# cshizhe/VLN-HAMT

Hardware: AMD Instinct MI355X
Metric: panorama-steps/sec, R2R proxy pretrain (36x768 views, 80-tok instr) (higher is better)
Workload: dtype bf16; 1 GPU; R2R 6-proxy-task pretrain step (fwd+bwd+clip+AdamW, dropout 0.1), fixed ViT features, R2R-canon model 174.8M params; per_gpu_batch=64, global_batch=64, txt_len=80, hist_len=5, views=36, task_mix=mlm:sap:sar:sprel:mrc:itm=5:1:1:1:2:2, parallelism=dp1, launch=hipGraph replay, dead_code_elimination=True

## Files before the change

### include/hamt.h

```cpp
#ifndef HAMT_H
#define HAMT_H

#include <stddef.h>
#include <stdint.h>

#ifdef __cplusplus
extern "C" {
#endif

#define HAMT_ABI_VERSION 2

typedef enum { HAMT_OK = 0, HAMT_ERR_ARG = -1, HAMT_ERR_UNSUPPORTED = -2, HAMT_ERR_LAUNCH = -3 } hamt_status;
typedef enum { HAMT_F32 = 0, HAMT_BF16 = 1,
               HAMT_U8G = 2,
               HAMT_F16 = 3 } hamt_dtype;
typedef enum { HAMT_PREC_BF16 = 0, HAMT_PREC_F32 = 1 } hamt_prec;

int hamt_version(void);
int hamt_last_error(char* buf, size_t n);
int hamt_last_kernel(char* buf, size_t n);
enum { HAMT_WS_GEMM_SPLITK = 0, HAMT_WS_COLSUM = 1, HAMT_WS_SUMSQ = 2, HAMT_WS_LN_BWD = 3, HAMT_WS_WGRAD_TABLE = 4, HAMT_WS_LNRED_TABLE = 5, HAMT_WS_VIS_EMBED_BWD = 6,
       HAMT_WS_EMBED_BWD = 7 ,
       HAMT_WS_OBJ_EMBED_BWD = 8, HAMT_WS_IMAGE_PREP = 9  };
size_t hamt_workspace_bytes(int op, const int* shape, int nshape);
// ... 196 lines not shown
  int layout;
  int ldy, dtype_y, Rpad;
} hamt_image_prep_desc;
int hamt_image_prep(const hamt_image_prep_desc* d, const hamt_image_view* views_host, const hamt_image_view* views_dev,
                    const uint8_t* src, const float* lut, void* y, void* ws, size_t ws_bytes, void* stream);
enum { HAMT_RESAMPLE_BICUBIC = 0 , HAMT_RESAMPLE_LANCZOS = 1  };
typedef struct {
  int n, H, W;
  int OH, OW;
  int x0, y0, w, h;
  int filter;
  int kx, ky;
} hamt_image_resample_desc;
int hamt_image_resample_taps(int in, int out, int filter, int first, int count, int32_t* xmin, int32_t* xcnt, int32_t* k, int ksize);
int hamt_image_resample(const hamt_image_resample_desc* d, const int32_t* xtab_host, const int32_t* ytab_host, const int32_t* xtab_dev,
                        const int32_t* ytab_dev, const uint8_t* src, uint8_t* dst, void* stream);
int hamt_add3(size_t n, const float* a, const float* b, const float* c, float* out, void* stream);
int hamt_dropout(size_t n, const float* x, float* y, float p, uint32_t call_id, const uint64_t* rng, void* stream);
int hamt_cast_f32_bf16(size_t n, const float* x, void* y, void* stream);
int hamt_unpack_padded(const void* src, const int32_t* prefix, int B, int maxlen, int row_bytes, int pad_byte, void* dst, void* stream);
int hamt_seq_masks(const int32_t* prefix, int add, int B, int maxlen, uint8_t* mask, int64_t* lens_out, void* stream);
int hamt_wire_pack_bf16(size_t n, const float* x, void* y, float scale, void* stream);
int hamt_wire_unpack_bf16(size_t n, const void* y, float* x, void* stream);
int hamt_fill_where_zero(size_t n, const int64_t* flag, float* x, float value, void* stream);
int hamt_extend_mask(size_t n, const void* mask_u8, float* out, void* stream);
int hamt_debug_fill_lds(uint32_t pattern, void* stream);
int hamt_debug_wgrad_timing(int on);
int hamt_debug_wgrad_times(float* us, int* tile_rows, double* flops, int cap);
int hamt_act_bwd(size_t n, const float* dy, const float* h, int mode, float* dx, void* stream);

int hamt_ce_fwd(int R, int C, const float* x, int ldx, const int64_t* label, float* loss, float* lse, void* stream);
int hamt_ce_bwd(int R, int C, const float* x, int ldx, const int64_t* label, const float* lse,
                const float* g, float* dx, int lddx, void* stream);
int hamt_mse_fwd(size_t n, const float* x, const float* t, float* loss, void* stream);
int hamt_mse_bwd(size_t n, const float* x, const float* t, const float* g, float* dx, void* stream);
int hamt_kl_fwd(int R, int C, const float* x, int ldx, const float* t, int ldt, float* loss, float* lse, void* stream);
int hamt_kl_bwd(int R, int C, const float* x, int ldx, const float* t, int ldt, const float* lse,
                const float* g, float* dx, int lddx, void* stream);
int hamt_eval_ce(int R, int C, const float* x, int ldx, const int64_t* label, float* ws, double* sums, int64_t* counts, void* stream);
int hamt_eval_kl(int R, int C, const float* x, int ldx, const float* t, int ldt, float* ws, double* sums, int64_t* counts,
                 void* stream);
int hamt_eval_mse_cols(int R, int C, const float* x, int ldx, const float* t, int ldt, double* sums, void* stream);
int hamt_a2c_fwd(int T, int B, const float* reward, const float* mask, const float* value, const float* logp, const float* ent,
                 const float* last_value, float gamma, float ent_w, float* ret, float* out, void* stream);
int hamt_a2c_bwd(int T, int B, const float* ret, const float* mask, const float* value, float ent_w, const float* g,
                 float* dlogp, float* dvalue, float* dent, void* stream);
#define HAMT_POLICY_TEACHER 0
#define HAMT_POLICY_ARGMAX 1
#define HAMT_POLICY_SAMPLE 2
int hamt_policy_step_fwd(int B, int V, int A, int mode, int64_t ignoreid, const float* logit, int ld_logit,
                         const int64_t* target, const uint8_t* bt_mask, const int32_t* cand_len, uint8_t* ended,
                         const float* ob_ang, const int64_t* forced_action, const float* uniform, const uint64_t* rng,
                         uint32_t call_id, float* ml, int64_t* action, float* logp, float* ent, float* mask,
                         int32_t* env_action, float* prev_angle, int32_t* hist_len, float* lse, void* stream);
int hamt_policy_step_bwd(int B, int V, int mode, int64_t ignoreid, const float* logit, int ld_logit, const int64_t* target,
                         const uint8_t* bt_mask, const int64_t* action, const float* lse, const float* g_ml,
                         const float* g_logp, const float* g_ent, int gs_ml, int gs_logp, int gs_ent, float* dlogit, int ld_dlogit,
                         void* stream);
#define HAMT_STOP_LOGIT_INDEX 0
#define HAMT_STOP_LOGIT_VALUE 1
int hamt_policy_ref_step_fwd(int B, int V, int O, int A, int mode, int stop_logit, int last_step, int64_t ignoreid,
                             const float* act_logit, int ld_act, const float* obj_logit, int ld_obj, const int32_t* obj_len,
                             const int32_t* cand_len, const int64_t* target, const int64_t* ref_target, const int32_t* obj_id,
                             const int32_t* goal_obj, const uint8_t* bt_mask, uint8_t* ended, const float* ob_ang,
                             const int64_t* forced_action, const float* uniform, const uint64_t* rng, uint32_t call_id,
                             float* ml, float* ref, int64_t* action, float* logp, float* ent, float* mask, int32_t* env_action,
// ... 90 lines not shown
```

### vln_hamt_amd/_lib.py

```python
from __future__ import annotations

import ctypes as C
import os

_HERE = os.path.dirname(os.path.abspath(__file__))
LIB_PATH = os.path.join(_HERE, "libhamt_hip.so")

HAMT_F32, HAMT_BF16, HAMT_U8G, HAMT_F16 = 0, 1, 2, 3
PREC_BF16, PREC_F32 = 0, 1
EPI_BIAS, EPI_GELU, EPI_RELU, EPI_ACCUM, EPI_MUL_DGELU, EPI_MUL_DRELU, EPI_SAVE_PRE = 1, 2, 4, 8, 16, 32, 64
EPI_GELU_GRAD, EPI_MUL_AUX, EPI_ADD_AUX, EPI_DROPOUT = 128, 256, 512, 1024
SUMSQ_SPARSE = 2
OPT_ADAMW, OPT_ADAM, OPT_RMSPROP, OPT_SGD = 0, 1, 2, 3

vp, i32, u32, f32, sz = C.c_void_p, C.c_int, C.c_uint32, C.c_float, C.c_size_t


class GemmDesc(C.Structure):
    _fields_ = [("M", i32), ("N", i32), ("K", i32), ("lda", i32), ("ldb", i32), ("ldc", i32), ("ldaux", i32),
                ("a_kmajor", i32), ("b_kmajor", i32), ("dtype_a", i32), ("dtype_b", i32), ("dtype_c", i32),
                ("dtype_aux", i32), ("prec", i32), ("epilogue", i32), ("alpha", f32), ("ka_rows", i32), ("kb_rows", i32),
                ("p_drop", f32), ("call_id", u32), ("rng", C.c_void_p)]


# ... 96 lines not shown
    "hamt_obj_embed_fwd": [C.POINTER(ObjEmbedDesc), C.POINTER(ObjEmbedParams)] + [vp] * 7,
    "hamt_obj_embed_bwd": [C.POINTER(ObjEmbedDesc), C.POINTER(ObjEmbedParams), C.POINTER(ObjEmbedGrads)] + [vp] * 10,
    "hamt_ln_fwd": [C.POINTER(LnDesc), vp, vp, vp, vp, vp, vp, vp, vp, vp, vp, vp],
    "hamt_ln_bwd": [C.POINTER(LnDesc), vp, vp, vp, vp, vp, vp, vp, vp, vp, vp, vp, vp, vp, vp],
    "hamt_ln_bwd_add": [C.POINTER(LnDesc), vp, vp, vp, vp, vp, vp, vp, vp, vp, vp, vp],
    "hamt_ln_bwd_reduce": [i32, i32, vp, vp, vp, vp, vp],
    "hamt_ln_bwd_reduce_grouped": [i32, vp, vp, sz, vp],
    "hamt_gather_rows": [i32, i32, vp, i32, vp, vp, i32, vp, i32, i32, vp],
    "hamt_scatter_add_rows": [i32, i32, vp, i32, i32, vp, vp, i32, vp],
    "hamt_scatter_add_rows_small": [i32, i32, vp, i32, i32, vp, i32, vp, vp, vp],
    "hamt_scatter_add_rows_ordered": [i32, i32, vp, i32, i32, vp, vp, i32, i32, vp, vp],
    "hamt_embed_sum_fwd": [i32, i32, i32, vp, vp, vp, vp, vp, vp],
    "hamt_embed_sum_bwd": [i32, i32, i32, i32, vp, vp, vp, vp, vp, vp, sz, vp],
    "hamt_mean_mid_fwd": [i32, i32, i32, vp, vp, vp],
    "hamt_mean_mid_bwd": [i32, i32, i32, vp, vp, vp],
    "hamt_mul_bcast_fwd": [i32, i32, i32, vp, vp, i32, vp, vp],
    "hamt_mul_bcast_bwd": [i32, i32, i32, vp, vp, i32, vp, vp, vp, vp],
    "hamt_sum_rows": [i32, i32, i32, vp, i32, vp, vp, vp],
    "hamt_patchify": [i32, i32, i32, i32, i32, vp, vp, i32, i32, i32, vp],
    "hamt_image_prep": [C.POINTER(ImagePrepDesc), vp, vp, vp, vp, vp, vp, sz, vp],
    "hamt_image_resample_taps": [i32, i32, i32, i32, i32, vp, vp, vp, i32],
    "hamt_image_resample": [C.POINTER(ImageResampleDesc), vp, vp, vp, vp, vp, vp, vp],
    "hamt_add3": [sz, vp, vp, vp, vp, vp],
    "hamt_dropout": [sz, vp, vp, f32, u32, vp, vp],
    "hamt_cast_f32_bf16": [sz, vp, vp, vp],
    "hamt_unpack_padded": [vp, vp, i32, i32, i32, i32, vp, vp],
    "hamt_seq_masks": [vp, i32, i32, i32, vp, vp, vp],
    "hamt_wire_pack_bf16": [C.c_size_t, vp, vp, f32, vp],
    "hamt_wire_unpack_bf16": [C.c_size_t, vp, vp, vp],
    "hamt_fill_where_zero": [sz, vp, vp, f32, vp],
    "hamt_act_bwd": [sz, vp, vp, i32, vp, vp],
    "hamt_ce_fwd": [i32, i32, vp, i32, vp, vp, vp, vp],
    "hamt_ce_bwd": [i32, i32, vp, i32, vp, vp, vp, vp, i32, vp],
    "hamt_mse_fwd": [sz, vp, vp, vp, vp],
    "hamt_mse_bwd": [sz, vp, vp, vp, vp, vp],
    "hamt_kl_fwd": [i32, i32, vp, i32, vp, i32, vp, vp, vp],
    "hamt_kl_bwd": [i32, i32, vp, i32, vp, i32, vp, vp, vp, i32, vp],
    "hamt_eval_ce": [i32, i32, vp, i32, vp, vp, vp, vp, vp],
    "hamt_eval_kl": [i32, i32, vp, i32, vp, i32, vp, vp, vp, vp],
    "hamt_eval_mse_cols": [i32, i32, vp, i32, vp, i32, vp, vp],
    "hamt_extend_mask": [sz, vp, vp, vp],
    "hamt_debug_fill_lds": [u32, vp],
    "hamt_debug_wgrad_timing": [C.c_int],
    "hamt_debug_wgrad_times": [vp, vp, vp, C.c_int],
    "hamt_a2c_fwd": [i32, i32, vp, vp, vp, vp, vp, vp, f32, f32, vp, vp, vp],
    "hamt_a2c_bwd": [i32, i32, vp, vp, vp, f32, vp, vp, vp, vp, vp],
    "hamt_policy_step_fwd": [i32, i32, i32, i32, C.c_int64, vp, i32] + [vp] * 8 + [u32] + [vp] * 10,
    "hamt_policy_step_bwd": [i32, i32, i32, C.c_int64, vp, i32] + [vp] * 7 + [i32, i32, i32, vp, i32, vp],
    "hamt_policy_ref_step_fwd": [i32] * 7 + [C.c_int64, vp, i32, vp, i32] + [vp] * 12 + [u32] + [vp] * 14,
    "hamt_policy_ref_step_bwd": [i32] * 5 + [vp, i32, vp, i32] + [vp] * 8 + [i32] * 4 + [vp, i32, vp, i32, vp],
    "hamt_nav_observe": [i32, i32, i32, i32, C.c_int64, i32, i32] + [vp] * 17,
    "hamt_nav_advance": [i32, i32, i32, i32] + [vp] * 19,
    "hamt_nav_eval": [i32, i32, i32] + [vp] * 10,
    "hamt_nav_advance_goals": [i32, i32, i32, i32] + [vp] * 15,
    "hamt_nav_advance_back": [i32, i32, i32, i32, i32] + [vp] * 23,
    "hamt_nav_eval_goals": [i32, i32, i32, i32] + [vp] * 12,
    "hamt_nav_eval_back": [i32, i32, i32] + [vp] * 12,
    "hamt_obs_gather": [i32, i32, i32, i32, i32, i32] + [vp] * 24,
    "hamt_obs_turn": [i32, i32] + [vp] * 5,
    "hamt_sumsq": [sz, vp, vp, i32, vp, vp],
    "hamt_sumsq_table": [sz, sz, vp, vp, vp, i32, vp, i32, vp, vp],
    "hamt_sumsq_partials": [sz, vp, vp, i32, vp],
    "hamt_wire_unpack_sumsq": [sz, sz, vp, vp, vp, vp, i32, vp, i32, vp, vp],
    "hamt_adamw_flat": [sz, vp, vp, vp, vp, vp, vp, vp, f32, f32, f32, f32, i32, vp],
    "hamt_adamw_table": [sz, vp, vp, vp, vp, vp, vp, vp, i32, vp, f32, f32, f32, f32, i32, vp],
    "hamt_adamw_table_range": [sz, sz, vp, vp, vp, vp, vp, vp, vp, i32, vp, f32, f32, f32, f32, i32, vp],
# ... 64 lines not shown
```

### vln_hamt_amd/csrc/gemm_epi.h

```cpp
#pragma once

template <int W> __device__ __forceinline__ void ld_bf(const bf16_t* p, float* o) {
  if constexpr (W == 8) {
    const uint4 u = *(const uint4*)p;
    const uint32_t w[4] = {u.x, u.y, u.z, u.w};
#pragma unroll
    for (int q = 0; q < 4; ++q) { o[2 * q] = __uint_as_float(w[q] << 16); o[2 * q + 1] = __uint_as_float(w[q] & 0xffff0000u); }
  } else {
    const uint2 u = *(const uint2*)p;
    o[0] = __uint_as_float(u.x << 16); o[1] = __uint_as_float(u.x & 0xffff0000u);
    o[2] = __uint_as_float(u.y << 16); o[3] = __uint_as_float(u.y & 0xffff0000u);
  }
}
template <int W> __device__ __forceinline__ void st_bf(bf16_t* p, const float* v) {
  if constexpr (W == 8) *(uint4*)p = make_uint4(pack_bf2(v[0], v[1]), pack_bf2(v[2], v[3]), pack_bf2(v[4], v[5]), pack_bf2(v[6], v[7]));
  else *(uint2*)p = make_uint2(pack_bf2(v[0], v[1]), pack_bf2(v[2], v[3]));
}
__device__ __forceinline__ uint32_t pack_16(float lo, float hi, bool f16) { return f16 ? pack_h2(lo, hi) : pack_bf2(lo, hi); }
__device__ __forceinline__ void unpack_16(uint32_t w, float& lo, float& hi, bool f16) {
  float a, b;
  unpack_h2(w, a, b);
  lo = f16 ? a : __uint_as_float(w << 16);
  hi = f16 ? b : __uint_as_float(w & 0xffff0000u);
}
// ... 105 lines not shown
    const bool ch = F16_OK && g.dtype_c == HAMT_F16;
    bf16_t* c = (bf16_t*)g.C + ic;
    if (vc) {
      if (epi & HAMT_EPI_ACCUM) { float p[W]; ld_16<W>(c, p, ch); _Pragma("unroll") for (int j = 0; j < W; ++j) v[j] += p[j]; }
      st_16<W>(c, v, ch);
    } else {
      _Pragma("unroll") for (int j = 0; j < W; ++j) if (col + j < g.N) {
        const float f = (epi & HAMT_EPI_ACCUM) ? v[j] + (ch ? h2f(c[j]) : bf2f(c[j])) : v[j];
        c[j] = ch ? f2h(f) : f2bf(f);
      }
    }
  } else {
    float* c = (float*)g.C + ic;
    if (vc) {
      if (epi & HAMT_EPI_ACCUM) {
        float p[W];
        if (W == 8 && pre_c && pre_ok) { _Pragma("unroll") for (int j = 0; j < 4; ++j) { p[j] = pre_c[0][j]; p[4 + j] = pre_c[1][j]; } }
        else ld_f<W>(c, p);
        _Pragma("unroll") for (int j = 0; j < W; ++j) v[j] += p[j];
      }
      st_f<W>(c, v);
      if (ssq) _Pragma("unroll") for (int j = 0; j < W; ++j) *ssq += v[j] * v[j];
    } else _Pragma("unroll") for (int j = 0; j < W; ++j) if (col + j < g.N) {
      const float f = (epi & HAMT_EPI_ACCUM) ? c[j] + v[j] : v[j];
      c[j] = f;
      if (ssq) *ssq += f * f;
    }
  }
}

constexpr int EPI_FAST_MASK = HAMT_EPI_BIAS | HAMT_EPI_GELU | HAMT_EPI_GELU_GRAD | HAMT_EPI_ACCUM | HAMT_EPI_MUL_AUX | HAMT_EPI_DROPOUT | HAMT_EPI_ADD_AUX;
__device__ __forceinline__ bool epi_fast_ok(const GemmArgsF& g, int epi, int m0, int n0, int bm, int bn) {
  (void)m0; (void)bm;
  bool ok = (epi & ~EPI_FAST_MASK) == 0 && g.ksplit <= 1 && n0 + bn <= g.N && (g.ldc & 7) == 0 && ((uintptr_t)g.C & 15) == 0;
  if (epi & HAMT_EPI_BIAS) ok = ok && ((uintptr_t)g.bias & 15) == 0;
  if (epi & (HAMT_EPI_GELU_GRAD | HAMT_EPI_MUL_AUX)) ok = ok && g.dtype_aux == HAMT_BF16 && (g.ldaux & 7) == 0 && ((uintptr_t)g.aux & 15) == 0;
  if (epi & HAMT_EPI_ADD_AUX)
    ok = ok && !(epi & (HAMT_EPI_GELU_GRAD | HAMT_EPI_MUL_AUX)) && (g.dtype_aux == HAMT_BF16 || g.dtype_aux == HAMT_F32) && (g.ldaux & 7) == 0 && ((uintptr_t)g.aux & 15) == 0;
  return ok;
}
template <int EPI, bool C16>
__device__ __forceinline__ void epi_fast8(const GemmArgsF& g, int row, int col, const float* acc, const float* b8, const uint4* pre_aux, float* ssq = nullptr) {
  if (row >= g.M) return;
  float v[8];
#pragma unroll
  for (int j = 0; j < 8; ++j) v[j] = (EPI & HAMT_EPI_BIAS) ? __builtin_fmaf(acc[j], g.alpha, b8[j]) : acc[j] * g.alpha;
  if constexpr ((EPI & HAMT_EPI_GELU) != 0) {
#pragma unroll
    for (int j = 0; j < 8; ++j) v[j] = gelu_erf(v[j]);
  }
  float keep[8];
  if constexpr ((EPI & HAMT_EPI_DROPOUT) != 0) {
    const RngKey key = rng_key(g.rng, g.call_id);
    const uint32_t rowh = hamt_mix32((uint32_t)row ^ key.k0);
    const float inv_keep = 1.0f / (1.0f - g.p_drop);
    float f0[4], f1[4];
    drop_scale4(key, rowh, (uint32_t)(col >> 2), g.p_drop, inv_keep, f0);
    drop_scale4(key, rowh, (uint32_t)(col >> 2) + 1u, g.p_drop, inv_keep, f1);
#pragma unroll
    for (int j = 0; j < 4; ++j) { keep[j] = f0[j]; keep[4 + j] = f1[j]; }
  }
  if constexpr ((EPI & HAMT_EPI_GELU_GRAD) != 0) {
    float dg[8];
#pragma unroll
    for (int j = 0; j < 8; ++j) gelu_and_grad(v[j], v[j], dg[j]);
    if constexpr ((EPI & HAMT_EPI_DROPOUT) != 0) {
#pragma unroll
      for (int j = 0; j < 8; ++j) dg[j] *= keep[j];
    }
    st_bf<8>((bf16_t*)g.aux + (size_t)row * g.ldaux + col, dg);
  }
// ... 40 lines not shown
```

### vln_hamt_amd/csrc/loss.hip

```cpp
#include "common.h"

namespace {

__device__ __forceinline__ float block_max(float v, float* red) {
  v = wave_max(v);
  if ((threadIdx.x & 63) == 0) red[threadIdx.x >> 6] = v;
  __syncthreads();
  v = fmaxf(fmaxf(red[0], red[1]), fmaxf(red[2], red[3]));
  __syncthreads();
  return v;
}
__device__ __forceinline__ float block_sum(float v, float* red) {
  v = wave_sum(v);
  if ((threadIdx.x & 63) == 0) red[threadIdx.x >> 6] = v;
  __syncthreads();
  v = (red[0] + red[1]) + (red[2] + red[3]);
  __syncthreads();
  return v;
}
__device__ __forceinline__ float row_lse(const float* x, int C, float* red) {
  float m = -INFINITY;
  for (int c = threadIdx.x; c < C; c += 256) m = fmaxf(m, x[c]);
  m = block_max(m, red);
  float s = 0.f;
  for (int c = threadIdx.x; c < C; c += 256) s += expf(x[c] - m);
  s = block_sum(s, red);
  return m + logf(s);
}

__global__ __launch_bounds__(256) void ce_fwd_kernel(int C, const float* __restrict__ x, int ldx, const int64_t* __restrict__ label,
                                                     float* __restrict__ loss, float* __restrict__ lse) {
  __shared__ float red[4];
  const int r = blockIdx.x;
  const float* xr = x + (size_t)r * ldx;
  const float l = row_lse(xr, C, red);
  if (threadIdx.x == 0) {
    const int64_t lab = label[r];
    lse[r] = l;
    loss[r] = lab < 0 ? 0.f : (lab < C ? l - xr[lab] : __builtin_nanf(""));
  }
}
__global__ __launch_bounds__(256) void ce_bwd_kernel(int C, const float* __restrict__ x, int ldx, const int64_t* __restrict__ label,
                                                     const float* __restrict__ lse, const float* __restrict__ g,
                                                     float* __restrict__ dx, int lddx) {
  const int r = blockIdx.x;
  const float* xr = x + (size_t)r * ldx;
  float* dr = dx + (size_t)r * lddx;
  const float l = lse[r], gr = g[r];
  const int64_t lab64 = label[r];
  const bool ignored = lab64 < 0;
  const float bad = lab64 >= C ? __builtin_nanf("") : 0.f;
  const int lab = (int)lab64;
  for (int c = threadIdx.x; c < C; c += 256) dr[c] = ignored ? 0.f : gr * (expf(xr[c] - l) - (c == lab ? 1.0f : 0.0f)) + bad;
}
__global__ void mse_fwd_kernel(size_t n, const float* __restrict__ x, const float* __restrict__ t, float* __restrict__ loss) {
  for (size_t i = (size_t)blockIdx.x * blockDim.x + threadIdx.x; i < n; i += (size_t)gridDim.x * blockDim.x) {
    const float d = x[i] - t[i];
    loss[i] = d * d;
  }
}
__global__ void mse_bwd_kernel(size_t n, const float* __restrict__ x, const float* __restrict__ t, const float* __restrict__ g,
                               float* __restrict__ dx) {
  for (size_t i = (size_t)blockIdx.x * blockDim.x + threadIdx.x; i < n; i += (size_t)gridDim.x * blockDim.x)
    dx[i] = 2.0f * g[i] * (x[i] - t[i]);
}
__global__ __launch_bounds__(256) void kl_fwd_kernel(int C, const float* __restrict__ x, int ldx, const float* __restrict__ t, int ldt,
                                                     float* __restrict__ loss, float* __restrict__ lse) {
  __shared__ float red[4];
  const int r = blockIdx.x;
  const float* xr = x + (size_t)r * ldx;
  const float* tr = t + (size_t)r * ldt;
  const float l = row_lse(xr, C, red);
  float s = 0.f;
  for (int c = threadIdx.x; c < C; c += 256) {
    const float tv = tr[c];
    s += (tv > 0.f ? tv * logf(tv) : 0.f) - tv * (xr[c] - l);
  }
  s = block_sum(s, red);
  if (threadIdx.x == 0) { loss[r] = s; lse[r] = l; }
}
__global__ __launch_bounds__(256) void kl_bwd_kernel(int C, const float* __restrict__ x, int ldx, const float* __restrict__ t, int ldt,
                                                     const float* __restrict__ lse, const float* __restrict__ g,
                                                     float* __restrict__ dx, int lddx) {
  __shared__ float red[4];
  const int r = blockIdx.x;
  const float* xr = x + (size_t)r * ldx;
// ... 10 lines not shown
                               const float* __restrict__ logp, const float* __restrict__ ent, const float* __restrict__ last_value,
                               float gamma, float ent_w, float* __restrict__ ret, float* __restrict__ out) {
  const int b = blockIdx.x * blockDim.x + threadIdx.x;
  if (b >= B) return;
  float R = last_value ? last_value[b] : 0.f, pol = 0.f, crit = 0.f, en = 0.f;
  for (int t = T - 1; t >= 0; --t) {
    const size_t i = (size_t)t * B + b;
    R = R * gamma + reward[i];
    ret[i] = R;
    const float a = R - value[i], m = mask[i];
    pol += -logp[i] * a * m;
    crit += 0.5f * a * a * m;
    if (ent) en += -ent_w * ent[i] * m;
  }
  out[3 * b] = pol; out[3 * b + 1] = crit; out[3 * b + 2] = en;
}
__global__ void a2c_bwd_kernel(size_t n, const float* __restrict__ ret, const float* __restrict__ mask, const float* __restrict__ value,
                               float ent_w, const float* __restrict__ g, float* __restrict__ dlogp, float* __restrict__ dvalue,
                               float* __restrict__ dent) {
  const float gs = *g;
  for (size_t i = (size_t)blockIdx.x * blockDim.x + threadIdx.x; i < n; i += (size_t)gridDim.x * blockDim.x) {
    const float a = ret[i] - value[i], m = mask[i];
    dlogp[i] = -a * m * gs;
    dvalue[i] = -a * m * gs;
    if (dent) dent[i] = -ent_w * m * gs;
  }
}

}

extern "C" int hamt_ce_fwd(int R, int C, const float* x, int ldx, const int64_t* label, float* loss, float* lse, void* stream) {
  if (R == 0) return HAMT_OK;
  HAMT_CHECK_ARG(x && label && loss && lse && C > 0, "hamt_ce_fwd: bad argument");
  hipLaunchKernelGGL(ce_fwd_kernel, dim3(R), dim3(256), 0, as_stream(stream), C, x, ldx, label, loss, lse);
  HAMT_CHECK_LAUNCH("hamt_ce_fwd");
  return HAMT_OK;
}
extern "C" int hamt_ce_bwd(int R, int C, const float* x, int ldx, const int64_t* label, const float* lse, const float* g,
                           float* dx, int lddx, void* stream) {
  if (R == 0) return HAMT_OK;
  HAMT_CHECK_ARG(x && label && lse && g && dx, "hamt_ce_bwd: null pointer");
  hipLaunchKernelGGL(ce_bwd_kernel, dim3(R), dim3(256), 0, as_stream(stream), C, x, ldx, label, lse, g, dx, lddx);
  HAMT_CHECK_LAUNCH("hamt_ce_bwd");
  return HAMT_OK;
}
extern "C" int hamt_mse_fwd(size_t n, const float* x, const float* t, float* loss, void* stream) {
  if (n == 0) return HAMT_OK;
  HAMT_CHECK_ARG(x && t && loss, "hamt_mse_fwd: null pointer");
  hipLaunchKernelGGL(mse_fwd_kernel, dim3(nb(n)), dim3(256), 0, as_stream(stream), n, x, t, loss);
  HAMT_CHECK_LAUNCH("hamt_mse_fwd");
  return HAMT_OK;
}
extern "C" int hamt_mse_bwd(size_t n, const float* x, const float* t, const float* g, float* dx, void* stream) {
  if (n == 0) return HAMT_OK;
  HAMT_CHECK_ARG(x && t && g && dx, "hamt_mse_bwd: null pointer");
  hipLaunchKernelGGL(mse_bwd_kernel, dim3(nb(n)), dim3(256), 0, as_stream(stream), n, x, t, g, dx);
  HAMT_CHECK_LAUNCH("hamt_mse_bwd");
  return HAMT_OK;
}
extern "C" int hamt_kl_fwd(int R, int C, const float* x, int ldx, const float* t, int ldt, float* loss, float* lse, void* stream) {
  if (R == 0) return HAMT_OK;
  HAMT_CHECK_ARG(x && t && loss && lse && C > 0, "hamt_kl_fwd: bad argument");
  hipLaunchKernelGGL(kl_fwd_kernel, dim3(R), dim3(256), 0, as_stream(stream), C, x, ldx, t, ldt, loss, lse);
  HAMT_CHECK_LAUNCH("hamt_kl_fwd");
  return HAMT_OK;
}
extern "C" int hamt_kl_bwd(int R, int C, const float* x, int ldx, const float* t, int ldt, const float* lse, const float* g,
                           float* dx, int lddx, void* stream) {
  if (R == 0) return HAMT_OK;
  HAMT_CHECK_ARG(x && t && lse && g && dx, "hamt_kl_bwd: null pointer");
  hipLaunchKernelGGL(kl_bwd_kernel, dim3(R), dim3(256), 0, as_stream(stream), C, x, ldx, t, ldt, lse, g, dx, lddx);
  HAMT_CHECK_LAUNCH("hamt_kl_bwd");
  return HAMT_OK;
}

extern "C" int hamt_a2c_fwd(int T, int B, const float* reward, const float* mask, const float* value, const float* logp, const float* ent,
// ... 17 lines not shown
```

### vln_hamt_amd/model/pretrain_cmt.py

```python
from __future__ import annotations

import os
from collections import defaultdict

import torch
from torch import nn

from .. import ops
from ..modeling import precision_of
from .vilmodel import BertLayerNorm, BertOnlyMLMHead, BertPreTrainedModel, NavPreTrainedModel


HEADS_FP32 = os.environ.get("HAMT_HEADS_BF16") is None
TXT_PACK = os.environ.get("HAMT_NO_TXT_PACK") is None


class _MlpHead(nn.Module):

    def __init__(self, in_size, hidden_size, out_size, dropout_rate=None, prec="bf16"):
        super().__init__()
        mods = [nn.Linear(in_size, hidden_size), nn.ReLU(), BertLayerNorm(hidden_size, eps=1e-12)]
        if dropout_rate is not None:
            mods.append(nn.Dropout(dropout_rate))
        mods.append(nn.Linear(hidden_size, out_size))
# ... 69 lines not shown

    def forward(self, batch, task, compute_loss=True):
        batch = defaultdict(lambda: None, batch)
        if batch['txt_ids'] is not None:
            pk = batch['txt_pack_idx']
            batch['txt_ids']._hamt_pack = (pk, batch['txt_cu'], batch['txt_unpack_idx']) if (pk is not None and TXT_PACK) else None
        hist = (batch['txt_ids'], batch['txt_masks'], batch['hist_img_fts'], batch['hist_ang_fts'],
                batch['hist_pano_img_fts'], batch['hist_pano_ang_fts'], batch['hist_masks'])
        ob = (batch['ob_img_fts'], batch['ob_ang_fts'], batch['ob_nav_types'], batch['ob_masks'])
        if task.startswith('mlm'):
            return self.forward_mlm(*hist, batch['txt_labels'], compute_loss, label_idx=batch['txt_label_idx'])
        elif task.startswith('sap'):
            return self.forward_sap(*hist, *ob, batch['ob_action_viewindex'], compute_loss)
        elif task.startswith('sar'):
            return self.forward_sar(*hist, *ob, batch['ob_action_angles'], batch['ob_progress'], compute_loss)
        elif task.startswith('sprel'):
            return self.forward_sprel(*hist, *ob, batch['sp_anchor_idxs'], batch['sp_targets'], compute_loss)
        elif task.startswith('mrc'):
            return self.forward_mrc(*hist, batch['hist_mrc_masks'], batch['hist_img_probs'], compute_loss,
                                    mrc_idx=batch['hist_mrc_idx'])
        elif task.startswith('itm'):
            return self.forward_itm(*hist, 4, compute_loss, neg_idxs=batch['itm_neg_idxs'],
                                    shuffled_pos_ids=batch['itm_shuffled_pos_ids'])
        else:
            raise ValueError('invalid task')

    def forward_mlm(self, txt_ids, txt_masks, hist_img_fts, hist_ang_fts, hist_pano_img_fts, hist_pano_ang_fts,
                    hist_masks, txt_labels, compute_loss, label_idx=None):
        if label_idx is None:
            label_idx = (txt_labels != -1).reshape(-1).nonzero(as_tuple=False).squeeze(1)
        txt_embeds, _, _ = self.bert(txt_ids, txt_masks, hist_img_fts, hist_ang_fts, hist_pano_img_fts,
                                     hist_pano_ang_fts, hist_masks, None, None, None, None, need="lang", lang_rows=label_idx)
        masked_output = txt_embeds if txt_embeds.dim() == 2 else ops.gather_rows(txt_embeds.reshape(-1, txt_embeds.size(-1)), label_idx, unique=True)
        prediction_scores = self.mlm_head(masked_output)
        if compute_loss:
            return ops.cross_entropy(prediction_scores, txt_labels.reshape(-1).index_select(0, label_idx))
        return prediction_scores

    def _compute_masked_hidden(self, hidden, mask):
        idx = mask.reshape(-1).nonzero(as_tuple=False).squeeze(1)
        return ops.gather_rows(hidden.reshape(-1, hidden.size(-1)), idx, unique=True)

    def forward_sap(self, txt_ids, txt_masks, hist_img_fts, hist_ang_fts, hist_pano_img_fts, hist_pano_ang_fts,
                    hist_masks, ob_img_fts, ob_ang_fts, ob_nav_types, ob_masks, act_labels, compute_loss):
        cls_rows = ops.const_index("arange_mul", int(txt_ids.size(0)), int(txt_ids.size(1)), device=txt_ids.device)
        txt_embeds, hist_embeds, ob_embeds = self.bert(txt_ids, txt_masks, hist_img_fts, hist_ang_fts,
                                                       hist_pano_img_fts, hist_pano_ang_fts, hist_masks,
                                                       ob_img_fts, ob_ang_fts, ob_nav_types, ob_masks, lang_rows=cls_rows)
        fused = ops.mul_bcast(ob_embeds, txt_embeds if txt_embeds.dim() == 2 else txt_embeds[:, 0])
        prediction_scores = self.next_action(fused).squeeze(-1)
        prediction_scores = ops.fill_where_zero(prediction_scores, ob_nav_types, -float('inf'))
        if compute_loss:
            return ops.cross_entropy(prediction_scores, act_labels)
        return prediction_scores

    def forward_sar(self, txt_ids, txt_masks, hist_img_fts, hist_ang_fts, hist_pano_img_fts, hist_pano_ang_fts,
                    hist_masks, ob_img_fts, ob_ang_fts, ob_nav_types, ob_masks, ob_act_angles, ob_progress, compute_loss):
        B, L = txt_ids.shape
        cls_rows = ops.const_index("arange_mul", int(B), int(L), device=txt_ids.device)
        txt_embeds, hist_embeds, ob_embeds = self.bert(txt_ids, txt_masks, hist_img_fts, hist_ang_fts,
                                                       hist_pano_img_fts, hist_pano_ang_fts, hist_masks,
                                                       ob_img_fts, ob_ang_fts, ob_nav_types, ob_masks, need="lang", lang_rows=cls_rows)
        cls = txt_embeds if txt_embeds.dim() == 2 else ops.gather_rows(txt_embeds.reshape(B * L, -1), cls_rows, unique=True)
        prediction_scores = self.regress_action(cls)
        if compute_loss:
            act_targets = torch.cat([ob_act_angles, ob_progress.unsqueeze(1)], dim=1)
# ... 46 lines not shown
```

### vln_hamt_amd/model/vilmodel.py

```python
from __future__ import annotations

import copy
import math
import os

import numpy as np
import torch
from torch import nn

from .. import blocks, ops, streams
from ..modeling import HamtPreTrainedModel, precision_of

BertLayerNorm = torch.nn.LayerNorm
BertPreTrainedModel = HamtPreTrainedModel

_ACT = {"gelu": ops.ACT_GELU, "relu": ops.ACT_RELU}


def gelu(x):
    return x * 0.5 * (1.0 + torch.erf(x / math.sqrt(2.0)))


def _p(drop: nn.Dropout, module: nn.Module) -> float:
    return float(drop.p) if module.training else 0.0
# ... 154 lines not shown
        if self.output_hidden_states:
            all_hidden += (hidden_states,)
        res = (hidden_states,)
        if self.output_hidden_states:
            res += (all_hidden,)
        if self.output_attentions:
            res += (all_att,)
        return res


class BertPredictionHeadTransform(nn.Module):

    def __init__(self, config):
        super().__init__()
        self.dense = nn.Linear(config.hidden_size, config.hidden_size)
        self.act = _act_code(config)
        self.LayerNorm = BertLayerNorm(config.hidden_size, eps=config.layer_norm_eps)
        self.prec = precision_of(config)

    def forward(self, hidden_states):
        h = ops.linear(hidden_states, self.dense.weight, self.dense.bias, self.act, self.prec)
        return ops.layer_norm(h, None, self.LayerNorm)


class BertLMPredictionHead(nn.Module):

    def __init__(self, config):
        super().__init__()
        self.transform = BertPredictionHeadTransform(config)
        self.decoder = nn.Linear(config.hidden_size, config.vocab_size, bias=False)
        self.bias = nn.Parameter(torch.zeros(config.vocab_size))
        self.prec = precision_of(config)

    def forward(self, hidden_states):
        h = self.transform(hidden_states)
        return ops.linear(h, self.decoder.weight, self.bias, ops.ACT_NONE, self.prec)


class BertOnlyMLMHead(nn.Module):

    def __init__(self, config):
        super().__init__()
        self.predictions = BertLMPredictionHead(config)

    def forward(self, sequence_output):
        return self.predictions(sequence_output)


class BertOutAttention(nn.Module):

    def __init__(self, config, ctx_dim=None):
        super().__init__()
        if config.hidden_size % config.num_attention_heads != 0:
            raise ValueError("The hidden size (%d) is not a multiple of the number of attention heads (%d)"
                             % (config.hidden_size, config.num_attention_heads))
        self.num_attention_heads = config.num_attention_heads
        self.attention_head_size = int(config.hidden_size / config.num_attention_heads)
        self.all_head_size = self.num_attention_heads * self.attention_head_size
        if ctx_dim is None:
            ctx_dim = config.hidden_size
        self.query = nn.Linear(config.hidden_size, self.all_head_size)
        self.key = nn.Linear(ctx_dim, self.all_head_size)
        self.value = nn.Linear(ctx_dim, self.all_head_size)
        self.dropout = nn.Dropout(config.attention_probs_dropout_prob)
        self.prec = precision_of(config)

    def forward(self, hidden_states, context, attention_mask=None):
        B, Sq, H = hidden_states.shape
        q = ops.linear(hidden_states.reshape(B * Sq, H), self.query.weight, self.query.bias, ops.ACT_NONE, self.prec)
        kv = ops.packed_linear(context, self.prec, self.key, self.value)
        ctx = ops.attention(q, kv, attention_mask, B, self.num_attention_heads, _p(self.dropout, self), self.prec)
        return ctx.view(B, Sq, H)


class BertXAttention(nn.Module):

    def __init__(self, config, ctx_dim=None):
        super().__init__()
        self.att = BertOutAttention(config, ctx_dim=ctx_dim)
# ... 421 lines not shown
```

### vln_hamt_amd/ops.py

```python
from __future__ import annotations

import ctypes as C
import math
import os
from typing import Optional

import torch

from . import _lib as L

_rng_state = {}
_call_counter = [0]


def rng_state(device) -> torch.Tensor:
    d = torch.device(device)
    key = d.index
    if key is None:
        key = torch.cuda.current_device() if d.type == "cuda" else 0
    t = _rng_state.get(key)
    if t is None:
        t = torch.tensor([0x243F6A8885A308D3 & 0x7FFFFFFFFFFFFFFF, 0], dtype=torch.int64,
                         device=torch.device(d.type, key) if d.type == "cuda" else d)
        _rng_state[key] = t
# ... 1123 lines not shown


class KlFn(torch.autograd.Function):

    @staticmethod
    def forward(ctx, x, t):
        _chk(x, "KlFn")
        assert x.dim() == 2
        if x.stride(1) != 1:
            x = x.contiguous()
        t = t.contiguous().to(torch.float32)
        R, Cc = x.shape
        loss = torch.empty(R, dtype=torch.float32, device=x.device)
        lse = torch.empty(R, dtype=torch.float32, device=x.device)
        L.check(L.load().hamt_kl_fwd(R, Cc, _p(x), x.stride(0), _p(t), Cc, _p(loss), _p(lse), _stream()), "hamt_kl_fwd")
        ctx.save_for_backward(x, t, lse)
        return loss

    @staticmethod
    def backward(ctx, g):
        x, t, lse = ctx.saved_tensors
        R, Cc = x.shape
        g = g.contiguous()
        ld = (Cc + 7) // 8 * 8
        buf = torch.empty(R, ld, dtype=torch.float32, device=x.device)
        L.check(L.load().hamt_kl_bwd(R, Cc, _p(x), x.stride(0), _p(t), Cc, _p(lse), _p(g), _p(buf), ld, _stream()), "hamt_kl_bwd")
        return buf[:, :Cc], None


def cross_entropy(x, label):
    return CrossEntropyFn.apply(x, label)


def mse_loss(x, t):
    return MseFn.apply(x, t)


class A2cFn(torch.autograd.Function):
    @staticmethod
    def forward(ctx, logp, value, ent, reward, mask, last_value, gamma, ent_w):
        T, B = logp.shape
        dev = logp.device
        f = lambda t: None if t is None else t.detach().to(torch.float32).contiguous()
        logp_, value_, ent_, reward_, mask_, last_ = f(logp), f(value), f(ent), f(reward), f(mask), f(last_value)
        ret = torch.empty(T, B, dtype=torch.float32, device=dev)
        out = torch.empty(B, 3, dtype=torch.float32, device=dev)
        L.check(L.load().hamt_a2c_fwd(T, B, _p(reward_), _p(mask_), _p(value_), _p(logp_), _p(ent_), _p(last_), float(gamma), float(ent_w),
                                      _p(ret), _p(out), _stream()), "hamt_a2c_fwd")
        ctx.save_for_backward(ret, mask_, value_)
        ctx.meta = (T, B, float(ent_w), ent is not None)
        return out

    @staticmethod
    def backward(ctx, dout):
        ret, mask_, value_ = ctx.saved_tensors
        T, B, ent_w, has_ent = ctx.meta
        dev = ret.device
        g = dout.reshape(-1)[:1].to(torch.float32).contiguous()
        dlogp = torch.empty(T, B, dtype=torch.float32, device=dev)
        dvalue = torch.empty(T, B, dtype=torch.float32, device=dev)
        dent = torch.empty(T, B, dtype=torch.float32, device=dev) if has_ent else None
        L.check(L.load().hamt_a2c_bwd(T, B, _p(ret), _p(mask_), _p(value_), ent_w, _p(g), _p(dlogp), _p(dvalue), _p(dent), _stream()), "hamt_a2c_bwd")
        return dlogp, dvalue, dent, None, None, None, None, None


def a2c_loss(logp, value, reward, mask, last_value=None, entropy=None, gamma=0.9, entropy_weight=0.01, normalize="total"):
# ... 403 lines not shown
```

Baseline: 6642 panorama-steps/s.

## Fuse MLM head linear with cross-entropy and emit bf16 logit gradients directly

Adds an MlmHeadLossFn path that runs the vocab projection, CE forward and a new CE backward kernel that writes bf16 padded dy directly. The dy then feeds the dgrad GEMM and the deferred wgrad queue, skipping the fp32 dy buffer and a separate cast when possible. It also adds a register-resident single-pass CE forward kernel for large vocabularies and relaxes the fp32 ldc alignment check in the GEMM fast epilogue. The gain is less memory traffic over the 30k-wide logits, at the cost of extra code paths and a dependency on weight tying holding.

```diff
diff --git a/include/hamt.h b/include/hamt.h
--- a/include/hamt.h
+++ b/include/hamt.h
@@ -252,6 +252,8 @@
 int hamt_ce_fwd(int R, int C, const float* x, int ldx, const int64_t* label, float* loss, float* lse, void* stream);
 int hamt_ce_bwd(int R, int C, const float* x, int ldx, const int64_t* label, const float* lse,
                 const float* g, float* dx, int lddx, void* stream);
+int hamt_ce_bwd16(int R, int C, const float* x, int ldx, const int64_t* label, const float* lse, const float* g,
+                  float* dx, int lddx, void* y, int ldy, int Rpad, int Cpad, void* stream);
 int hamt_mse_fwd(size_t n, const float* x, const float* t, float* loss, void* stream);
 int hamt_mse_bwd(size_t n, const float* x, const float* t, const float* g, float* dx, void* stream);
 int hamt_kl_fwd(int R, int C, const float* x, int ldx, const float* t, int ldt, float* loss, float* lse, void* stream);
diff --git a/vln_hamt_amd/_lib.py b/vln_hamt_amd/_lib.py
--- a/vln_hamt_amd/_lib.py
+++ b/vln_hamt_amd/_lib.py
@@ -152,6 +152,7 @@
     "hamt_act_bwd": [sz, vp, vp, i32, vp, vp],
     "hamt_ce_fwd": [i32, i32, vp, i32, vp, vp, vp, vp],
     "hamt_ce_bwd": [i32, i32, vp, i32, vp, vp, vp, vp, i32, vp],
+    "hamt_ce_bwd16": [i32, i32, vp, i32, vp, vp, vp, vp, i32, vp, i32, i32, i32, vp],
     "hamt_mse_fwd": [sz, vp, vp, vp, vp],
     "hamt_mse_bwd": [sz, vp, vp, vp, vp, vp],
     "hamt_kl_fwd": [i32, i32, vp, i32, vp, i32, vp, vp, vp],
diff --git a/vln_hamt_amd/csrc/gemm_epi.h b/vln_hamt_amd/csrc/gemm_epi.h
--- a/vln_hamt_amd/csrc/gemm_epi.h
+++ b/vln_hamt_amd/csrc/gemm_epi.h
@@ -161,11 +161,12 @@
 constexpr int EPI_FAST_MASK = HAMT_EPI_BIAS | HAMT_EPI_GELU | HAMT_EPI_GELU_GRAD | HAMT_EPI_ACCUM | HAMT_EPI_MUL_AUX | HAMT_EPI_DROPOUT | HAMT_EPI_ADD_AUX;
 __device__ __forceinline__ bool epi_fast_ok(const GemmArgsF& g, int epi, int m0, int n0, int bm, int bn) {
   (void)m0; (void)bm;
-  bool ok = (epi & ~EPI_FAST_MASK) == 0 && g.ksplit <= 1 && n0 + bn <= g.N && (g.ldc & 7) == 0 && ((uintptr_t)g.C & 15) == 0;
+  const int cmask = g.dtype_c == HAMT_F32 ? 3 : 7, amask = g.dtype_aux == HAMT_F32 ? 3 : 7;
+  bool ok = (epi & ~EPI_FAST_MASK) == 0 && g.ksplit <= 1 && n0 + bn <= g.N && (g.ldc & cmask) == 0 && ((uintptr_t)g.C & 15) == 0;
   if (epi & HAMT_EPI_BIAS) ok = ok && ((uintptr_t)g.bias & 15) == 0;
   if (epi & (HAMT_EPI_GELU_GRAD | HAMT_EPI_MUL_AUX)) ok = ok && g.dtype_aux == HAMT_BF16 && (g.ldaux & 7) == 0 && ((uintptr_t)g.aux & 15) == 0;
   if (epi & HAMT_EPI_ADD_AUX)
-    ok = ok && !(epi & (HAMT_EPI_GELU_GRAD | HAMT_EPI_MUL_AUX)) && (g.dtype_aux == HAMT_BF16 || g.dtype_aux == HAMT_F32) && (g.ldaux & 7) == 0 && ((uintptr_t)g.aux & 15) == 0;
+    ok = ok && !(epi & (HAMT_EPI_GELU_GRAD | HAMT_EPI_MUL_AUX)) && (g.dtype_aux == HAMT_BF16 || g.dtype_aux == HAMT_F32) && (g.ldaux & amask) == 0 && ((uintptr_t)g.aux & 15) == 0;
   return ok;
 }
 template <int EPI, bool C16>
diff --git a/vln_hamt_amd/csrc/loss.hip b/vln_hamt_amd/csrc/loss.hip
--- a/vln_hamt_amd/csrc/loss.hip
+++ b/vln_hamt_amd/csrc/loss.hip
@@ -40,6 +40,38 @@
     loss[r] = lab < 0 ? 0.f : (lab < C ? l - xr[lab] : __builtin_nanf(""));
   }
 }
+template <int NV>
+__global__ __launch_bounds__(256) void ce_fwd_row_kernel(int C, const float* __restrict__ x, int ldx, const int64_t* __restrict__ label,
+                                                         float* __restrict__ loss, float* __restrict__ lse) {
+  __shared__ float red[4];
+  const int r = blockIdx.x, t = threadIdx.x;
+  const float* xr = x + (size_t)r * ldx;
+  float v[NV];
+#pragma unroll
+  for (int k = 0; k < NV; ++k) {
+    const int c = t + 256 * k;
+    v[k] = c < C ? xr[c] : -INFINITY;
+  }
+  float m = -INFINITY;
+#pragma unroll
+  for (int k = 0; k < NV; ++k) m = fmaxf(m, v[k]);
+  m = block_max(m, red);
+  float s = 0.f;
+#pragma unroll
+  for (int k = 0; k < NV; ++k) s += expf(v[k] - m);
+  s = block_sum(s, red);
+  if (t == 0) {
+    const float l = m + logf(s);
+    const int64_t lab = label[r];
+    lse[r] = l;
+    loss[r] = lab < 0 ? 0.f : (lab < C ? l - xr[lab] : __builtin_nanf(""));
+  }
+}
+constexpr int CE_ROW_NV = 128, CE_ROW_MIN_C = 1024;
+
+__device__ __forceinline__ float ce_grad(float xv, float l, float gr, bool hit, bool ignored, float bad) {
+  return ignored ? 0.f : gr * (expf(xv - l) - (hit ? 1.0f : 0.0f)) + bad;
+}
 __global__ __launch_bounds__(256) void ce_bwd_kernel(int C, const float* __restrict__ x, int ldx, const int64_t* __restrict__ label,
                                                      const float* __restrict__ lse, const float* __restrict__ g,
                                                      float* __restrict__ dx, int lddx) {
@@ -51,7 +83,41 @@
   const bool ignored = lab64 < 0;
   const float bad = lab64 >= C ? __builtin_nanf("") : 0.f;
   const int lab = (int)lab64;
-  for (int c = threadIdx.x; c < C; c += 256) dr[c] = ignored ? 0.f : gr * (expf(xr[c] - l) - (c == lab ? 1.0f : 0.0f)) + bad;
+  for (int c = threadIdx.x; c < C; c += 256) dr[c] = ce_grad(xr[c], l, gr, c == lab, ignored, bad);
+}
+template <bool DX>
+__global__ __launch_bounds__(256) void ce_bwd16_kernel(int R, int C, int Cpad, const float* __restrict__ x, int ldx, const int64_t* __restrict__ label,
+                                                       const float* __restrict__ lse, const float* __restrict__ g,
+                                                       float* __restrict__ dx, int lddx, bf16_t* __restrict__ y, int ldy) {
+  const int r = blockIdx.x, t = threadIdx.x;
+  bf16_t* yr = y + (size_t)r * ldy;
+  if (r >= R) {
+    for (int c = 8 * t; c < Cpad; c += 8 * 256) *(uint4*)(yr + c) = make_uint4(0u, 0u, 0u, 0u);
+    return;
+  }
+  const float* xr = x + (size_t)r * ldx;
+  float* dr = DX ? dx + (size_t)r * lddx : nullptr;
+  const float l = lse[r], gr = g[r];
+  const int64_t lab64 = label[r];
+  const bool ignored = lab64 < 0;
+  const float bad = lab64 >= C ? __builtin_nanf("") : 0.f;
+  const int lab = (int)lab64;
+  const bool vec = (((uintptr_t)xr) & 15) == 0 && (!DX || (((uintptr_t)dr) & 15) == 0);
+  const int c8 = vec ? (C >> 3) << 3 : 0;
+  for (int c = 8 * t; c < c8; c += 8 * 256) {
+    const float4 a = *(const float4*)(xr + c), b = *(const float4*)(xr + c + 4);
+    const float xs[8] = {a.x, a.y, a.z, a.w, b.x, b.y, b.z, b.w};
+    float d[8];
+#pragma unroll
+    for (int j = 0; j < 8; ++j) d[j] = ce_grad(xs[j], l, gr, c + j == lab, ignored, bad);
+    if constexpr (DX) { *(float4*)(dr + c) = make_float4(d[0], d[1], d[2], d[3]); *(float4*)(dr + c + 4) = make_float4(d[4], d[5], d[6], d[7]); }
+    *(uint4*)(yr + c) = make_uint4(pack_bf2(d[0], d[1]), pack_bf2(d[2], d[3]), pack_bf2(d[4], d[5]), pack_bf2(d[6], d[7]));
+  }
+  for (int c = c8 + t; c < Cpad; c += 256) {
+    const float d = c < C ? ce_grad(xr[c], l, gr, c == lab, ignored, bad) : 0.f;
+    if constexpr (DX) { if (c < C) dr[c] = d; }
+    yr[c] = f2bf(d);
+  }
 }
 __global__ void mse_fwd_kernel(size_t n, const float* __restrict__ x, const float* __restrict__ t, float* __restrict__ loss) {
   for (size_t i = (size_t)blockIdx.x * blockDim.x + threadIdx.x; i < n; i += (size_t)gridDim.x * blockDim.x) {
@@ -128,7 +194,11 @@
 extern "C" int hamt_ce_fwd(int R, int C, const float* x, int ldx, const int64_t* label, float* loss, float* lse, void* stream) {
   if (R == 0) return HAMT_OK;
   HAMT_CHECK_ARG(x && label && loss && lse && C > 0, "hamt_ce_fwd: bad argument");
-  hipLaunchKernelGGL(ce_fwd_kernel, dim3(R), dim3(256), 0, as_stream(stream), C, x, ldx, label, loss, lse);
+  static const bool two_pass = getenv("HAMT_CE_TWO_PASS") != nullptr;
+  if (C >= CE_ROW_MIN_C && C <= 256 * CE_ROW_NV && !two_pass)
+    hipLaunchKernelGGL(ce_fwd_row_kernel<CE_ROW_NV>, dim3(R), dim3(256), 0, as_stream(stream), C, x, ldx, label, loss, lse);
+  else
+    hipLaunchKernelGGL(ce_fwd_kernel, dim3(R), dim3(256), 0, as_stream(stream), C, x, ldx, label, loss, lse);
   HAMT_CHECK_LAUNCH("hamt_ce_fwd");
   return HAMT_OK;
 }
@@ -138,6 +208,17 @@
   HAMT_CHECK_ARG(x && label && lse && g && dx, "hamt_ce_bwd: null pointer");
   hipLaunchKernelGGL(ce_bwd_kernel, dim3(R), dim3(256), 0, as_stream(stream), C, x, ldx, label, lse, g, dx, lddx);
   HAMT_CHECK_LAUNCH("hamt_ce_bwd");
+  return HAMT_OK;
+}
+extern "C" int hamt_ce_bwd16(int R, int C, const float* x, int ldx, const int64_t* label, const float* lse, const float* g,
+                             float* dx, int lddx, void* y, int ldy, int Rpad, int Cpad, void* stream) {
+  if (Rpad == 0 && R == 0) return HAMT_OK;
+  HAMT_CHECK_ARG(R >= 0 && C > 0 && Rpad >= R && Cpad >= C && Cpad % 8 == 0 && ldy >= Cpad && ldy % 8 == 0 && y && ((uintptr_t)y & 15) == 0,
+                 "hamt_ce_bwd16: bad argument");
+  HAMT_CHECK_ARG(R == 0 || (x && label && lse && g && ldx >= C && (!dx || lddx >= C)), "hamt_ce_bwd16: bad argument");
+  if (dx) hipLaunchKernelGGL(ce_bwd16_kernel<true>, dim3(Rpad), dim3(256), 0, as_stream(stream), R, C, Cpad, x, ldx, label, lse, g, dx, lddx, (bf16_t*)y, ldy);
+  else hipLaunchKernelGGL(ce_bwd16_kernel<false>, dim3(Rpad), dim3(256), 0, as_stream(stream), R, C, Cpad, x, ldx, label, lse, g, dx, lddx, (bf16_t*)y, ldy);
+  HAMT_CHECK_LAUNCH("hamt_ce_bwd16");
   return HAMT_OK;
 }
 extern "C" int hamt_mse_fwd(size_t n, const float* x, const float* t, float* loss, void* stream) {
diff --git a/vln_hamt_amd/model/pretrain_cmt.py b/vln_hamt_amd/model/pretrain_cmt.py
--- a/vln_hamt_amd/model/pretrain_cmt.py
+++ b/vln_hamt_amd/model/pretrain_cmt.py
@@ -125,6 +125,8 @@
         txt_embeds, _, _ = self.bert(txt_ids, txt_masks, hist_img_fts, hist_ang_fts, hist_pano_img_fts,
                                      hist_pano_ang_fts, hist_masks, None, None, None, None, need="lang", lang_rows=label_idx)
         masked_output = txt_embeds if txt_embeds.dim() == 2 else ops.gather_rows(txt_embeds.reshape(-1, txt_embeds.size(-1)), label_idx, unique=True)
+        if compute_loss and self.mlm_head.predictions.decoder.weight is self.bert.embeddings.word_embeddings.weight:
+            return self.mlm_head(masked_output, txt_labels.reshape(-1).index_select(0, label_idx))
         prediction_scores = self.mlm_head(masked_output)
         if compute_loss:
             return ops.cross_entropy(prediction_scores, txt_labels.reshape(-1).index_select(0, label_idx))
diff --git a/vln_hamt_amd/model/vilmodel.py b/vln_hamt_amd/model/vilmodel.py
--- a/vln_hamt_amd/model/vilmodel.py
+++ b/vln_hamt_amd/model/vilmodel.py
@@ -210,8 +210,10 @@
         self.bias = nn.Parameter(torch.zeros(config.vocab_size))
         self.prec = precision_of(config)
 
-    def forward(self, hidden_states):
+    def forward(self, hidden_states, labels=None):
         h = self.transform(hidden_states)
+        if labels is not None:
+            return ops.mlm_head_loss(h, self.decoder.weight, self.bias, labels, self.prec)
         return ops.linear(h, self.decoder.weight, self.bias, ops.ACT_NONE, self.prec)
 
 
@@ -221,8 +223,8 @@
         super().__init__()
         self.predictions = BertLMPredictionHead(config)
 
-    def forward(self, sequence_output):
-        return self.predictions(sequence_output)
+    def forward(self, sequence_output, labels=None):
+        return self.predictions(sequence_output, labels)
 
 
 class BertOutAttention(nn.Module):
diff --git a/vln_hamt_amd/ops.py b/vln_hamt_amd/ops.py
--- a/vln_hamt_amd/ops.py
+++ b/vln_hamt_amd/ops.py
@@ -1179,6 +1179,60 @@
     return CrossEntropyFn.apply(x, label)
 
 
+MLM_CHAIN = os.environ.get("HAMT_NO_MLM_CHAIN") is None
+
+
+class MlmHeadLossFn(torch.autograd.Function):
+
+    @staticmethod
+    def forward(ctx, h, weight, bias, label):
+        _chk(h, "MlmHeadLossFn")
+        x2 = h if h.stride(-1) == 1 else h.contiguous()
+        M, N = x2.shape[0], weight.shape[0]
+        x16 = prep_x16(x2, "bf16")
+        logits = empty_rows(M, N, h.device)
+        _linear_fwd(x2, weight, bias.detach(), logits, ACT_NONE, "bf16", None, x16)
+        label = label.contiguous()
+        loss = torch.empty(M, dtype=torch.float32, device=h.device)
+        lse = torch.empty(M, dtype=torch.float32, device=h.device)
+        L.check(L.load().hamt_ce_fwd(M, N, _p(logits), logits.stride(0), _p(label), _p(loss), _p(lse), _stream()), "hamt_ce_fwd")
+        ctx.save_for_backward(x16, weight, logits, label, lse)
+        ctx.bias_param = bias if bias.is_leaf else False
+        return loss
+
+    @staticmethod
+    def backward(ctx, g):
+        from . import wgrad
+        x16, weight, logits, label, lse = ctx.saved_tensors
+        M, N = logits.shape
+        K = weight.shape[1]
+        need_dx, need_dw, need_db = ctx.needs_input_grad[:3]
+        g = g.contiguous()
+        dy16 = torch.empty(x16.shape[0], _rup(N), dtype=torch.bfloat16, device=g.device)
+        queued = need_dw and ctx.bias_param is not False and wgrad.eligible(weight, dy16[:, :N], x16)
+        lean = queued or not (need_dw or need_db)
+        dy32 = None if lean else torch.empty(M, (N + 7) // 8 * 8, dtype=torch.float32, device=g.device)
+        L.check(L.load().hamt_ce_bwd16(M, N, _p(logits), logits.stride(0), _p(label), _p(lse), _p(g), _p(dy32), dy32.stride(0) if dy32 is not None else 0,
+                                       _p(dy16), dy16.stride(0), dy16.shape[0], dy16.shape[1], _stream()), "hamt_ce_bwd16")
+        if not lean:
+            dx, dw, db = _linear_bwd(dy32[:, :N], None, x16, weight, "bf16", need_dx, need_dw, need_db, dy16=dy16, bias_param=ctx.bias_param)
+            return dx, dw, db, None
+        dx = None
+        if need_dx:
+            dx = torch.empty(M, K, dtype=torch.float32, device=g.device)
+            gemm(dy16[:M], weight_operand(weight, "bf16"), dx, b_kmajor=True, prec="bf16", k_red=dy16.shape[1])
+        if queued:
+            wgrad.defer(weight, ctx.bias_param if need_db else None, dy16[:, :N], x16)
+        return dx, None, None, None
+
+
+def mlm_head_loss(h, weight, bias, label, prec="bf16"):
+    if (MLM_CHAIN and prec == "bf16" and h.is_cuda and h.dim() == 2 and h.dtype == torch.float32 and _fast_ok(h.shape[1])
+            and bias is not None and weight.dtype == torch.float32):
+        return MlmHeadLossFn.apply(h, weight, bias, label)
+    return cross_entropy(linear(h, weight, bias, ACT_NONE, prec), label)
+
+
 def mse_loss(x, t):
     return MseFn.apply(x, t)
 
```

Measured after the change: 6670 panorama-steps/s, median of 6. About the same (+0.4%).
